# byronknoll/gmix

Measured on AMD Instinct MI355X. Metric: mixer bits/sec (synthetic 256-input mixer streams, forward+update), higher is better.
Workload: dtype f32; 1 GPU; configs[1]: synthetic 256-input 1-layer mixer (1 mixer, 2^16-row gate table), random logits, forward+update; n_inputs=256, mixers=1/0/0, streams_per_gpu=4096, total_bits=5486149632, parallelism=streams sharded over 1 GPU(s), no collective on the data path

## Files before the change

gmix_amd/csrc/gmx_capi.cpp:

```cpp
#include <hip/hip_runtime.h>
#include <math.h>
#include <stdio.h>
#include <stdlib.h>
#include <string.h>
#include <time.h>

#include <algorithm>
#include <atomic>
#include <map>
#include <new>
#include <string>
#include <vector>

#include "../../include/gmxmix.h"
#include "gmx_buildhash.h"
#include "gmx_internal.h"
#include "gmx_ckpt.h"
#include "gmx_ind_ckpt.h"
#include "gmx_match.h"
#include "gmx_match_ckpt.h"

struct GmxSynthArgs {
  float* pred;
  uint32_t* mask;
  uint32_t* ctx;
  uint8_t* bits;
  uint64_t* rng;
  uint64_t* tcount;
  float* pstate;
  uint32_t* cstate;
  uint64_t rec_stride, n_bits, seed;
  int32_t n, n_pad, m, mask_words, n_streams, restart, ctx_mode, bit_mode;
  uint32_t ctx_mod, zero_mod;
};

extern "C" {
hipError_t gmx_launch_bank_kernel(const GmxTopoDev* tp_dev, const GmxRunArgs* args, int n_streams,
                                  unsigned lds_bytes, int has_mask, int l0, int l1, int ns, int fin,
                                  unsigned stride0, hipStream_t stream);
hipError_t gmx_bank_kernel_set_lds(unsigned lds_bytes);
int gmx_bank_kernel_build(int l0, int l1, int ns, int fin, unsigned stride0);
hipError_t gmx_launch_stock_kernel(const GmxTopoDev* tp_dev, const GmxRunArgs* args, int n_streams,
                                   unsigned lds_bytes, int has_mask, int staged, int pow2_tables, hipStream_t stream);
hipError_t gmx_launch_single_kernel(const GmxTopoDev* tp_dev, const GmxRunArgs* args, int n_inputs,
                                    int variant, hipStream_t stream);
hipError_t gmx_launch_wide_kernel(const GmxTopoDev* tp_dev, const GmxRunArgs* args, int n_streams, int has_mask,
                                  int n_inputs, hipStream_t stream);
hipError_t gmx_launch_pair_kernel(const GmxTopoDev* tp_dev, const GmxRunArgs* args, int n_streams, int has_mask,
                                  int n_inputs, int l0, int l1, hipStream_t stream);
int gmx_pair_kernel_half(int n_inputs);
hipError_t gmx_launch_synth_kernel(const GmxSynthArgs* args, hipStream_t stream);
struct GmxDecayArgs {
  const uint64_t* steps0;
  float* table;
  uint32_t* amb;
  uint32_t amb_cap, U;
  uint64_t T;
};
hipError_t gmx_launch_decay_kernel(const GmxDecayArgs* args, hipStream_t stream);
hipError_t gmx_launch_init_scal(uint8_t* banks, uint64_t bank_bytes, uint64_t scal_off, int m,
                                int n_streams, hipStream_t stream);
hipError_t gmx_launch_math_probe(const float* x, float* y, uint64_t n, int what, hipStream_t stream);
hipError_t gmx_launch_math_range(uint64_t lo, uint64_t count, int what, unsigned long long* out,
                                 hipStream_t stream);
}

static thread_local std::string g_last_error;

static int hip_fail(hipError_t e, const char* what) {
  char buf[512];
  snprintf(buf, sizeof buf, "%s: %s (%d)", what, hipGetErrorString(e), (int)e);
  g_last_error = buf;
  (void)hipGetLastError();
  return GMX_ERR_HIP;
}
#define HIPCHK(call)                                   \
  do {                                                 \
    hipError_t e_ = (call);                            \
    if (e_ != hipSuccess) return hip_fail(e_, #call);  \
  } while (0)

static const size_t kBatchOwnStreamMin = 256u * 1024u;
struct GmxXfer {
  hipEvent_t ev_up = nullptr;
  hipEvent_t ev_dev = nullptr;
  hipEvent_t ev_down = nullptr;
  hipEvent_t ev_wr = nullptr;
  bool up_rec = false, dev_rec = false, down_rec = false, wr_rec = false;
  bool idle = false;
};
static int xfer_init(GmxXfer& x) {
  HIPCHK(hipEventCreateWithFlags(&x.ev_up, hipEventDisableTiming));
  HIPCHK(hipEventCreateWithFlags(&x.ev_dev, hipEventDisableTiming));
  HIPCHK(hipEventCreateWithFlags(&x.ev_down, hipEventDisableTiming));
  HIPCHK(hipEventCreateWithFlags(&x.ev_wr, hipEventDisableTiming));
  return GMX_OK;
}
static void xfer_free(GmxXfer& x) {
  hipEvent_t evs[] = {x.ev_up, x.ev_dev, x.ev_down, x.ev_wr};
  for (hipEvent_t e : evs)
    if (e) (void)hipEventDestroy(e);
  x = GmxXfer();
}
static int xfer_note_device_use(GmxXfer& x, hipStream_t main) {
  HIPCHK(hipEventRecord(x.ev_dev, main));
  x.dev_rec = true;
  x.idle = false;
  return GMX_OK;
}
static int xfer_writer_waits(GmxXfer& x, hipStream_t writer) {
  if (x.up_rec) HIPCHK(hipStreamWaitEvent(writer, x.ev_up, 0));
  if (x.dev_rec) HIPCHK(hipStreamWaitEvent(writer, x.ev_dev, 0));
  if (x.wr_rec) HIPCHK(hipStreamWaitEvent(writer, x.ev_wr, 0));
  return GMX_OK;
}
static int xfer_writer_done(GmxXfer& x, hipStream_t writer, hipStream_t main) {
  HIPCHK(hipEventRecord(x.ev_wr, writer));
  x.wr_rec = true;
  x.idle = false;
  HIPCHK(hipStreamWaitEvent(main, x.ev_wr, 0));
  return GMX_OK;
}
static hipError_t bank_stream_create(hipStream_t* out, int level ) {
  int least = 0, greatest = 0;
  hipError_t e = hipDeviceGetStreamPriorityRange(&least, &greatest);
  if (e != hipSuccess) return e;
  const int mid = (least + greatest) / 2;
  return hipStreamCreateWithPriority(out, hipStreamNonBlocking, level == 1 ? least : level == 2 ? greatest : mid);
}
static hipError_t sibling_stream_create(hipStream_t* out, hipStream_t main) {
// ... 83 lines not shown
  const int k = (int)(c.seq++ % (unsigned)kStageSlots);
  if (c.busy[k]) {
    HIPCHK(hipEventSynchronize(c.done[k]));
    c.busy[k] = false;
  }
  if ((size_t)n > c.cap) {
    for (int j = 0; j < kStageSlots; ++j) {
      if (c.busy[j]) {
        HIPCHK(hipEventSynchronize(c.done[j]));
        c.busy[j] = false;
      }
      if (c.dev[j]) (void)hipFree(c.dev[j]);
      if (c.host[j]) (void)hipHostFree(c.host[j]);
      c.dev[j] = nullptr;
      c.host[j] = nullptr;
    }
    c.cap = 0;
    const size_t cap = (size_t)n + 64;
    for (int j = 0; j < kStageSlots; ++j) {
      HIPCHK(hipMalloc((void**)&c.dev[j], cap * sizeof(uint64_t)));
      HIPCHK(hipHostMalloc((void**)&c.host[j], cap * sizeof(uint64_t), hipHostMallocDefault));
      if (!c.done[j]) HIPCHK(hipEventCreateWithFlags(&c.done[j], hipEventDisableTiming));
    }
    c.cap = cap;
  }
  memcpy(c.host[k], counts, (size_t)n * sizeof(uint64_t));
  HIPCHK(hipMemcpyAsync(c.dev[k], c.host[k], (size_t)n * sizeof(uint64_t), hipMemcpyHostToDevice, st));
  *dev_out = c.dev[k];
  return GMX_OK;
}
static int count_list_used(GmxCountList& c, hipStream_t st) {
  const int k = (int)((c.seq - 1u) % (unsigned)kStageSlots);
  HIPCHK(hipEventRecord(c.done[k], st));
  c.busy[k] = true;
  return GMX_OK;
}

struct gmx_group {
  int device = 0;
  int S = 0;
  GmxTopoDev topo;
  GmxTopoDev* topo_dev = nullptr;
  uint8_t* banks = nullptr;
  float* latch_out = nullptr;
  hipStream_t stream = nullptr;
  hipEvent_t ev0 = nullptr, ev1 = nullptr;
  unsigned lds_bytes = 0;
  std::vector<uint64_t> steps;
  std::vector<uint8_t> fwd_done;
  struct DecaySlot {
    float* dev = nullptr;
    uint32_t* idx_dev = nullptr;
    float* host = nullptr;
    uint32_t* idx_host = nullptr;
    size_t cap = 0;
    size_t idx_cap = 0;
    hipEvent_t done = nullptr;
    hipEvent_t ready = nullptr;
    bool busy = false;
    uint64_t* st_dev = nullptr;
    uint64_t* st_host = nullptr;
    uint32_t* amb_dev = nullptr;
    uint32_t* amb_host = nullptr;
    float* patch_host = nullptr;
    size_t st_cap = 0;
  } decay[kStageSlots];
  GmxCountList counts;
  hipStream_t copy_stream = nullptr;
  hipStream_t up_stream = nullptr, down_stream = nullptr;
  unsigned run_seq = 0;
  hipEvent_t tm0 = nullptr, tm1 = nullptr;
  gmx_batch* one = nullptr;
  std::vector<gmx_batch*> batches;
  std::vector<struct GmxSession*> sessions;
  std::vector<struct gmx_lockstep*> locksteps;
  bool banks_in_use_by_dead_kernel = false;
  bool use_sessions = true;
  bool mailbox_on_device = true;
  bool force_general = false;
  bool stock_exact = false;
  int stock_staged = -1;
  bool decay_on_host = false;
  bool stock_pairs = false;
  bool register_rows = false;
  int single_variant = 0;
  struct GmxCkptState* ckpt = nullptr;
};

struct gmx_batch {
  gmx_group* g = nullptr;
  int S = 0;
  uint64_t max_bits = 0;
  unsigned flags = 0;
  float* d_pred = nullptr;
  uint32_t* d_mask = nullptr;
  uint32_t* d_ctx = nullptr;
  uint8_t* d_bits = nullptr;
  float* d_p = nullptr;
  float* d_out = nullptr;
  float* d_last = nullptr;
  uint64_t* d_rng = nullptr;
  uint64_t* d_tcount = nullptr;
  float* d_pstate = nullptr;
  uint32_t* d_cstate = nullptr;
  float* h_pred = nullptr;
  uint32_t* h_mask = nullptr;
  uint32_t* h_ctx = nullptr;
  uint8_t* h_bits = nullptr;
  float* h_p = nullptr;
  float* h_out = nullptr;
  float* h_last = nullptr;
  GmxXfer x;
};

struct gmx_lockstep {
  gmx_group* g = nullptr;
  gmx_batch* b = nullptr;
  float* dec_host = nullptr;
  uint8_t* bits_host = nullptr;
  float* dec_dev = nullptr;
  uint32_t* idx_dev = nullptr;
  hipGraph_t g_predict = nullptr, g_learn = nullptr, g_step = nullptr;
  hipGraphExec_t x_predict = nullptr, x_learn = nullptr, x_step = nullptr;
  bool predicted = false;
  bool persistent = false, ps_running = false, ps_dead = false, ps_counted = false;
  hipStream_t ps_stream = nullptr;
  GmxLsDoor* door = nullptr;
  uint32_t* done = nullptr;
  uint32_t* blk_seen = nullptr;
  uint32_t* blk_replay = nullptr;
  uint32_t* relay = nullptr;
  float* live = nullptr;
  uint32_t seq = 0, word = 0, completed = 0;
  bool learn_inflight = false;
};

enum GmxKernelKind : int;
static GmxKernelKind kernel_for(const gmx_group* g, unsigned mode);
static int sessions_close(gmx_group* g, bool keep_forward);
static int locksteps_stop(gmx_group* g, gmx_lockstep* except, bool keep_forward);
static void sessions_free(gmx_group* g);
static void ckpt_free(gmx_group* g);

extern "C" const char* gmx_strerror(int status) {
  switch (status) {
    case GMX_OK: return "ok";
    case GMX_ERR_INVALID: return "invalid argument or unsupported topology";
    case GMX_ERR_NOMEM: return "out of memory";
    case GMX_ERR_HIP: return "HIP runtime error";
    case GMX_ERR_NO_DEVICE: return "no usable gfx950 device (this library has no CPU fallback)";
    case GMX_ERR_STATE: return "call order violated";
    case GMX_ERR_FORMAT: return "malformed checkpoint";
    default: return "unknown status";
  }
}

extern "C" const char* gmx_last_error(void) { return g_last_error.c_str(); }

extern "C" const char* gmx_build_info(void) {
  return "libgmxmix gfx950 (CDNA4) hipcc -O3 -ffp-contract=off; abi 1; src " GMX_SRC_HASH "; kernels " GMX_KERN_HASH;
}

extern "C" int gmx_device_count(int* count) {
  if (!count) return GMX_ERR_INVALID;
  int n = 0;
  hipError_t e = hipGetDeviceCount(&n);
// ... 392 lines not shown
    on_device = rcd == GMX_OK;
  }
  if (!on_device) {
    for (auto& kv : uniq) {
      float* tab = d.host + (size_t)kv.second * T;
      if (learn)
        for (uint64_t t = 0; t < T; ++t) tab[t] = decay_base(kv.first + t);
      else
        for (uint64_t t = 0; t < T; ++t) tab[t] = 0.f;
    }
    HIPCHK(hipMemcpyAsync(d.dev, d.host, uniq.size() * T * sizeof(float), hipMemcpyHostToDevice, g->copy_stream));
  }
  memcpy(d.idx_host, idx.data(), ns * sizeof(uint32_t));
  HIPCHK(hipMemcpyAsync(d.idx_dev, d.idx_host, ns * sizeof(uint32_t), hipMemcpyHostToDevice, g->copy_stream));
  HIPCHK(hipEventRecord(d.ready, g->copy_stream));
  HIPCHK(hipStreamWaitEvent(g->stream, d.ready, 0));
  return GMX_OK;
}

static bool topo_register_rows_eligible(const GmxTopoDev& t) {
  return t.has_final && t.l0 >= 1 && t.l0 <= 24 && t.l1 >= 1 && t.l1 <= 8 && t.m == t.l0 + t.l1 + 1 &&
         t.n_skip == 1 && gmx_pair_kernel_half(t.n) != 0;
}

enum GmxKernelKind : int { GMX_K_SINGLE, GMX_K_WIDE, GMX_K_STOCK, GMX_K_BANK, GMX_K_PAIR };
static GmxKernelKind kernel_for(const gmx_group* g, unsigned mode) {
  if (g->register_rows && (mode & GMX_MODE_PREDICT) && !(mode & GMX_MODE_LATCH) && !g->force_general &&
      topo_register_rows_eligible(g->topo))
    return GMX_K_PAIR;
  const bool single = g->topo.m == 1 && g->topo.n <= 256 && (mode & GMX_MODE_PREDICT) &&
                      !(mode & GMX_MODE_LATCH) && !g->force_general;
  const bool stock = g->topo.n == 90 && g->topo.l0 == 24 && g->topo.l1 == 8 && g->topo.n_skip == 1 &&
                     g->topo.has_final && g->topo.mx[23].stride == 128 && !g->force_general;
  const bool wide = g->topo.l0 == 24 && g->topo.l1 == 8 && g->topo.n_skip == 1 && g->topo.has_final &&
                    ((g->topo.n == 256 && g->topo.mx[23].stride == 288) ||
                     (g->topo.n == 90 && g->topo.mx[23].stride == 128 && g->stock_pairs && !g->stock_exact)) &&
                    (mode & GMX_MODE_PREDICT) && !(mode & GMX_MODE_LATCH) && !g->force_general;
  return single ? GMX_K_SINGLE : wide ? GMX_K_WIDE : stock ? GMX_K_STOCK : GMX_K_BANK;
}

static int launch_run(gmx_group* g, gmx_batch* b, int s0, int rec0, int ns, uint64_t T,
                      unsigned mode, float* kernel_ms, const uint64_t* n_list = nullptr) {
  if (T == 0) return GMX_OK;
  for (gmx_lockstep* ls : g->locksteps) ls->predicted = false;
  gmx_group::DecaySlot* dec = nullptr;
  int rc = prepare_decay(g, s0, ns, T, (mode & GMX_MODE_LEARN) ? 1 : 0, &dec);
  if (rc) return rc;
  GmxRunArgs a;
  memset(&a, 0, sizeof a);
  a.banks = g->banks;
  a.pred = b->d_pred;
  a.mask = (b->flags & GMX_BATCH_MASK) ? b->d_mask : nullptr;
  a.ctx = b->d_ctx;
  a.bits = b->d_bits;
  a.decay = dec->dev;
  a.decay_idx = dec->idx_dev;
  a.p_out = b->d_p;
  a.out_all = (b->flags & GMX_BATCH_OUTPUTS) ? b->d_out : nullptr;
  a.out_last = (b->flags & GMX_BATCH_LAST_OUTPUTS) ? b->d_last : nullptr;
  a.latch_out = g->latch_out;
  a.rec_stride = b->max_bits;
  a.T = T;
  if (n_list) {
    int rcl = count_list_stage(g->counts, n_list, ns, g->stream, &a.T_list);
    if (rcl) return rcl;
  }
  a.mode = mode | (g->stock_exact ? GMX_MODE_EXACT : 0u);
  a.stream_base = s0;
  a.rec_base = rec0;
  a.n_streams = ns;
  {
    int rcx = xfer_before_run(b->x, g->stream);
    if (rcx) return rcx;
  }
  if (kernel_ms) HIPCHK(hipEventRecord(g->ev0, g->stream));
  const GmxKernelKind kind = kernel_for(g, mode);
  const bool single = kind == GMX_K_SINGLE, wide = kind == GMX_K_WIDE, stock = kind == GMX_K_STOCK;
  if (a.out_last && (single || wide)) return GMX_ERR_INVALID;
  if (kind == GMX_K_PAIR)
    HIPCHK(gmx_launch_pair_kernel(g->topo_dev, &a, ns, a.mask != nullptr, g->topo.n, g->topo.l0, g->topo.l1, g->stream));
  else if (single)
    HIPCHK(gmx_launch_single_kernel(g->topo_dev, &a, g->topo.n, g->single_variant, g->stream));
  else if (wide)
    HIPCHK(gmx_launch_wide_kernel(g->topo_dev, &a, ns, a.mask != nullptr, g->topo.n, g->stream));
  else if (stock)
    HIPCHK(gmx_launch_stock_kernel(g->topo_dev, &a, ns, GMX_STK_LDS_BYTES(g->topo.lds_misc),
                                   a.mask != nullptr, g->stock_staged, topo_tables_pow2(g->topo), g->stream));
  else
    HIPCHK(gmx_launch_bank_kernel(g->topo_dev, &a, ns, g->lds_bytes, a.mask != nullptr, g->topo.l0,
                                  g->topo.l1, g->topo.n_skip, g->topo.has_final,
                                  g->topo.mx[g->topo.l0 - 1].stride, g->stream));
  HIPCHK(hipEventRecord(dec->done, g->stream));
  dec->busy = true;
  if (n_list) {
    int rcl = count_list_used(g->counts, g->stream);
    if (rcl) return rcl;
  }
  {
    int rcn = batch_note_device_use(b);
    if (rcn) return rcn;
  }
  if (kernel_ms) {
    HIPCHK(hipEventRecord(g->ev1, g->stream));
    HIPCHK(hipEventSynchronize(g->ev1));
    HIPCHK(hipEventElapsedTime(kernel_ms, g->ev0, g->ev1));
  }
  if (mode & GMX_MODE_LEARN)
    for (int i = 0; i < ns; ++i) g->steps[s0 + i] += n_list ? n_list[i] : T;
  return GMX_OK;
}

static void batch_free(gmx_batch* b) {
  if (!b) return;
  if (b->g) {
    (void)hipSetDevice(b->g->device);
    if (b->g->stream) (void)hipStreamSynchronize(b->g->stream);
    if (b->g->up_stream) (void)hipStreamSynchronize(b->g->up_stream);
    if (b->g->down_stream) (void)hipStreamSynchronize(b->g->down_stream);
    auto& v = b->g->batches;
    v.erase(std::remove(v.begin(), v.end(), b), v.end());
  }
  void* dv[] = {b->d_pred, b->d_mask, b->d_ctx, b->d_bits, b->d_p, b->d_out, b->d_last,
                b->d_rng, b->d_tcount, b->d_pstate, b->d_cstate};
  for (void* p : dv)
    if (p) (void)hipFree(p);
  void* hv[] = {b->h_pred, b->h_mask, b->h_ctx, b->h_bits, b->h_p, b->h_out, b->h_last};
  for (void* p : hv)
    if (p) (void)hipHostFree(p);
  xfer_free(b->x);
  delete b;
}

static int batch_alloc(gmx_batch** out, gmx_group* g, int S, uint64_t max_bits, unsigned flags) {
  if (!out || !g || max_bits == 0) return GMX_ERR_INVALID;
  *out = nullptr;
  HIPCHK(hipSetDevice(g->device));
  gmx_batch* b = new (std::nothrow) gmx_batch();
  if (!b) return GMX_ERR_NOMEM;
  b->g = g;
  b->S = S;
  b->max_bits = max_bits;
  b->flags = flags;
  const GmxTopoDev& t = g->topo;
  const size_t R = (size_t)S * max_bits;
#define BCHK(call)                                 \
  do {                                             \
    hipError_t e_ = (call);                        \
    if (e_ != hipSuccess) {                        \
      int r_ = hip_fail(e_, #call);                \
      batch_free(b);                               \
      return e_ == hipErrorOutOfMemory ? GMX_ERR_NOMEM : r_; \
    }                                              \
  } while (0)
  BCHK(hipMalloc((void**)&b->d_pred, R * t.n_pad * sizeof(float)));
  if (flags & GMX_BATCH_MASK) BCHK(hipMalloc((void**)&b->d_mask, R * t.mask_words * sizeof(uint32_t)));
  BCHK(hipMalloc((void**)&b->d_ctx, (R + 1) * t.m * sizeof(uint32_t)));
  BCHK(hipMalloc((void**)&b->d_bits, R));
  BCHK(hipMalloc((void**)&b->d_p, R * sizeof(float)));
  if (flags & GMX_BATCH_OUTPUTS) BCHK(hipMalloc((void**)&b->d_out, R * t.m * sizeof(float)));
  if (flags & GMX_BATCH_LAST_OUTPUTS) {
    BCHK(hipMalloc((void**)&b->d_last, (size_t)S * t.m * sizeof(float)));
    BCHK(hipMemset(b->d_last, 0, (size_t)S * t.m * sizeof(float)));
  }
#undef BCHK
  {
    int rcx = xfer_init(b->x);
    if (rcx) {
// ... 371 lines not shown
      memcpy(w + (size_t)r * x.stride, p + 12, 4 * (size_t)input_size);
      p += 12 + 4 * (size_t)input_size;
    }
  }
  if (p != end) return GMX_ERR_FORMAT;
  HIPCHK(hipSetDevice(g->device));
  int rc = sessions_close(g, true);
  if (rc) return rc;
  if (stream < (int)g->sessions.size() && g->sessions[stream]) g->sessions[stream]->fwd_live = false;
  HIPCHK(hipStreamSynchronize(g->stream));
  HIPCHK(hipMemcpy(g->banks + (size_t)stream * t.bank_bytes, img.data(), img.size(),
                   hipMemcpyHostToDevice));
  g->steps[stream] = sc[0];
  g->fwd_done[stream] = 0;
  for (gmx_lockstep* ls : g->locksteps) ls->predicted = false;
  return GMX_OK;
}

extern "C" int gmx_bank_copy(gmx_group* dst, int dst_stream, gmx_group* src, int src_stream) {
  if (!dst || !src || dst_stream < 0 || dst_stream >= dst->S || src_stream < 0 || src_stream >= src->S)
    return GMX_ERR_INVALID;
  const GmxTopoDev &a = dst->topo, &b = src->topo;
  if (a.m != b.m || a.n != b.n || a.n_skip != b.n_skip || a.bank_bytes != b.bank_bytes)
    return GMX_ERR_INVALID;
  for (int j = 0; j < a.m; ++j)
    if (a.mx[j].table_size != b.mx[j].table_size || a.mx[j].weight_size != b.mx[j].weight_size ||
        a.mx[j].layer != b.mx[j].layer)
      return GMX_ERR_INVALID;
  HIPCHK(hipSetDevice(src->device));
  int rc = sessions_close(src, true);
  if (rc) return rc;
  HIPCHK(hipStreamSynchronize(src->stream));
  HIPCHK(hipSetDevice(dst->device));
  rc = sessions_close(dst, true);
  if (rc) return rc;
  if (dst_stream < (int)dst->sessions.size() && dst->sessions[dst_stream])
    dst->sessions[dst_stream]->fwd_live = false;
  HIPCHK(hipStreamSynchronize(dst->stream));
  HIPCHK(hipMemcpy(dst->banks + (size_t)dst_stream * a.bank_bytes,
                   src->banks + (size_t)src_stream * b.bank_bytes, a.bank_bytes,
                   hipMemcpyDeviceToDevice));
  dst->steps[dst_stream] = src->steps[src_stream];
  dst->fwd_done[dst_stream] = 0;
  for (gmx_lockstep* ls : dst->locksteps) ls->predicted = false;
  return GMX_OK;
}

#include "gmx_ckpt.inc"

extern "C" int gmx_bank_memory_usage(gmx_group* g, int stream, int mixer, uint64_t* bytes) {
  if (!g || stream < 0 || stream >= g->S || mixer < 0 || mixer >= g->topo.m || !bytes)
    return GMX_ERR_INVALID;
  HIPCHK(hipSetDevice(g->device));
  int rc = sessions_close(g, true);
  if (rc) return rc;
  HIPCHK(hipStreamSynchronize(g->stream));
  uint64_t sc[3];
  HIPCHK(hipMemcpy(sc, g->banks + (size_t)stream * g->topo.bank_bytes + g->topo.scal_off + 24u * mixer,
                   24, hipMemcpyDeviceToHost));
  const GmxMixerDev& x = g->topo.mx[mixer];
  *bytes = 29 + sc[2] * (uint64_t)(x.weight_size * 4 + 12) + 8ull * x.table_size;
  return GMX_OK;
}


#include "gmx_indirect.inc"
#include "gmx_ind_ckpt.inc"
#include "gmx_lstm.inc"
#include "gmx_match.inc"
#include "gmx_match_ckpt.inc"
#include "gmx_chainstep.inc"

extern "C" int gmx_debug_single_variant(gmx_group* g, int lanes_per_stream) {
  if (!g || (lanes_per_stream != 0 && lanes_per_stream != 16 && lanes_per_stream != 32 &&
             lanes_per_stream != 64 && lanes_per_stream != 165 && lanes_per_stream != 325))
    return GMX_ERR_INVALID;
  g->single_variant = lanes_per_stream;
  return GMX_OK;
}

extern "C" int gmx_debug_stock_pairs(gmx_group* g, int on) {
  if (!g) return GMX_ERR_INVALID;
  g->stock_pairs = on != 0;
  return GMX_OK;
}

extern "C" int gmx_debug_decay_on_host(gmx_group* g, int on) {
  if (!g) return GMX_ERR_INVALID;
  g->decay_on_host = on != 0;
  return GMX_OK;
}

extern "C" int gmx_debug_decay_table(gmx_group* g, const uint64_t* steps0, int U, uint64_t T, float* out,
                                     uint32_t* n_unsettled) {
  if (!g || !steps0 || U < 1 || T < 1 || !out) return GMX_ERR_INVALID;
  HIPCHK(hipSetDevice(g->device));
  if (!g->copy_stream) HIPCHK(sibling_stream_create(&g->copy_stream, g->stream));
  gmx_group::DecaySlot tmp;
  std::map<uint64_t, uint32_t> uniq;
  std::vector<uint32_t> row(U);
  for (int u = 0; u < U; ++u) {
    auto it = uniq.find(steps0[u]);
    if (it == uniq.end()) it = uniq.emplace(steps0[u], (uint32_t)uniq.size()).first;
    row[u] = it->second;
  }
  HIPCHK(hipMalloc((void**)&tmp.dev, uniq.size() * T * sizeof(float)));
  int rc = decay_table_on_device(g, tmp, uniq, T);
  if (rc == GMX_OK) {
    if (n_unsettled) *n_unsettled = tmp.amb_host[0];
    std::vector<float> h(uniq.size() * T);
    hipError_t e = hipMemcpyAsync(h.data(), tmp.dev, h.size() * sizeof(float), hipMemcpyDeviceToHost, g->copy_stream);
    if (e == hipSuccess) e = hipStreamSynchronize(g->copy_stream);
    if (e != hipSuccess) rc = hip_fail(e, "gmx_debug_decay_table copy");
    else
      for (int u = 0; u < U; ++u) memcpy(out + (size_t)u * T, h.data() + (size_t)row[u] * T, T * sizeof(float));
  }
  void* dv[] = {tmp.dev, tmp.st_dev, tmp.amb_dev};
  for (void* p : dv)
    if (p) (void)hipFree(p);
  void* hv[] = {tmp.st_host, tmp.amb_host, tmp.patch_host};
  for (void* p : hv)
    if (p) (void)hipHostFree(p);
  return rc;
}

extern "C" int gmx_topology_register_rows_eligible(const gmx_topology* topo) {
  GmxTopoDev td;
  if (build_topology(topo, &td) != GMX_OK) return GMX_ERR_INVALID;
  return topo_register_rows_eligible(td) ? 1 : 0;
}

extern "C" int gmx_group_set_register_rows(gmx_group* g, int on) {
  if (!g || !topo_register_rows_eligible(g->topo)) return GMX_ERR_INVALID;
  g->register_rows = on != 0;
  return GMX_OK;
}

extern "C" int gmx_debug_force_general(gmx_group* g, int on) {
  if (!g) return GMX_ERR_INVALID;
  g->force_general = on != 0;
  return GMX_OK;
}

extern "C" int gmx_debug_kernel_kind(gmx_group* g, unsigned mode) {
  if (!g) return GMX_ERR_INVALID;
  const GmxKernelKind kind = kernel_for(g, mode);
  if (kind != GMX_K_BANK) return (int)kind;
  const GmxTopoDev& t = g->topo;
  return (int)kind + 4 * gmx_bank_kernel_build(t.l0, t.l1, t.n_skip, t.has_final, t.mx[t.l0 - 1].stride);
}

extern "C" int gmx_debug_stock_staged(gmx_group* g, int mode) {
  if (!g || mode < -1 || mode > 1) return GMX_ERR_INVALID;
  g->stock_staged = mode;
  return GMX_OK;
}

extern "C" int gmx_debug_stock_exact(gmx_group* g, int on) {
  if (!g) return GMX_ERR_INVALID;
  int rc = sessions_close(g, true);
  if (rc) return rc;
  g->stock_exact = on != 0;
  return GMX_OK;
}

extern "C" int gmx_debug_use_sessions(gmx_group* g, int on) {
// ... 404 lines not shown
```

gmix_amd/csrc/gmx_wide.hip:

```cpp
#include <hip/hip_runtime.h>
#include <stdint.h>

#include "gmx_internal.h"
#include "gmx_math.h"

typedef float gmx_f4 __attribute__((ext_vector_type(4)));

namespace {

constexpr int kL0 = 24, kL1 = 8, kM = kL0 + kL1 + 1;
constexpr int kQS = 9;
constexpr int kFinLane = 56;
constexpr int kPitchS = 4 * kQS + 4;

template <int N, int HALF>
struct WideShape {
  static constexpr int kN = N, kHalf = HALF;
  static constexpr int kNPad = (N + 3) / 4 * 4;
  static constexpr int kMW = (N + 31) / 32;
  static constexpr int kQ = HALF / 4;
  static constexpr int kUp = N - HALF;
  static constexpr int kQU = (kUp + 3) / 4;
  static constexpr int kPitch = HALF + 4;
  static constexpr int kStageSmall = 2 * kL0 * kPitch;
  static constexpr int kStageFloats = kStageSmall + (kL1 + 1) * kPitchS;
  static_assert(HALF % 4 == 0 && HALF <= N && N - HALF + kL0 - 1 <= HALF, "layer-0 rows must split into two lanes");
  static_assert((kPitch / 4) % 2 == 1, "odd quad pitch keeps the transposed reads conflict-free");
  static constexpr int stage_off(int h) {
    return h < kL0 ? h * kPitch
           : h < 32 ? kStageSmall + (h - kL0) * kPitchS
           : h < 32 + kL0 ? (kL0 + h - 32) * kPitch
           : h == kFinLane ? kStageSmall + kL1 * kPitchS : 0;
  }
  static constexpr int stage_lanes(int h) {
    return h < kL0 ? kQ : (h >= 32 && h < 32 + kL0) ? (kUp + (h - 32) + 3) / 4 : ((h < 32 || h == kFinLane) ? kQS : 0);
  }
};

__device__ __forceinline__ void wide_ld16(gmx_f4& d, const void* p) {
  asm volatile("global_load_dwordx4 %0, %1, off nt" : "=v"(d) : "v"(p) : "memory");
}
__device__ __forceinline__ void wide_ld4(uint32_t& d, const void* p) {
  asm volatile("global_load_dword %0, %1, off" : "=v"(d) : "v"(p) : "memory");
}
__device__ __forceinline__ void wide_ld1(uint32_t& d, const void* p) {
  asm volatile("global_load_ubyte %0, %1, off" : "=v"(d) : "v"(p) : "memory");
}
__device__ __forceinline__ uint32_t readlane_u(uint32_t v, int l) {
  return (uint32_t)__builtin_amdgcn_readlane((int)v, l);
}
__device__ __forceinline__ uint32_t wide_lds_addr(const void* p) {
  return (uint32_t)(uintptr_t)(__attribute__((address_space(3))) const void*)p;
}
__device__ __forceinline__ void wide_dma16(uint64_t sbase, uint32_t voff, uint32_t lds_byte, uint64_t mask) {
  uint32_t sm0;
  asm volatile(
      "s_mov_b64 exec, %3\n\ts_mov_b32 %0, m0\n\ts_mov_b32 m0, %4\n\ts_nop 0\n\t"
      "global_load_lds_dwordx4 %2, %1 nt\n\ts_mov_b32 m0, %0\n\ts_mov_b64 exec, -1"
      : "=&s"(sm0)
      : "s"(sbase), "v"(voff), "s"(mask), "s"(lds_byte)
      : "memory");
}
__device__ __forceinline__ void wide_st16(uint64_t sbase, uint32_t voff, const gmx_f4& v, uint64_t mask) {
  asm volatile(
      "s_mov_b64 exec, %3\n\t"
      "global_store_dwordx4 %1, %2, %0 nt\n\ts_mov_b64 exec, -1"
      :
      : "s"(sbase), "v"(voff), "v"(v), "s"(mask)
      : "memory");
}
__device__ __forceinline__ float readlane_f(float v, int l) {
  return __int_as_float(__builtin_amdgcn_readlane(__float_as_int(v), l));
}
__device__ __forceinline__ float el(const gmx_f4& v, int e) { return e == 0 ? v.x : (e == 1 ? v.y : (e == 2 ? v.z : v.w)); }

}

template <int N, int HALF, bool HAS_MASK>
__global__ void __launch_bounds__(64) __attribute__((amdgpu_waves_per_eu(1, 2)))
gmx_wide_kernel(const GmxTopoDev* __restrict__ tp, const GmxRunArgs a) {
  using SH = WideShape<N, HALF>;
  constexpr int kHalf = SH::kHalf, kNPad = SH::kNPad, kMW = SH::kMW, kQ = SH::kQ, kUp = SH::kUp,
                kQU = SH::kQU, kPitch = SH::kPitch, kStageSmall = SH::kStageSmall;
  __shared__ __attribute__((aligned(16))) float xin[kNPad + 4];
  __shared__ __attribute__((aligned(16))) float stage[SH::kStageFloats];
  __shared__ uint64_t s_tab[32];
  const int lane = threadIdx.x;
  const int rec = a.rec_base + (int)blockIdx.x;
  const int s = a.stream_base + (int)blockIdx.x;
  const uint64_t T = a.T;
  if (T == 0) return;
  if (lane < 32) s_tab[lane] = gmx_exp2f_tab[lane];
  for (int i = 4 * lane; i < SH::kStageFloats; i += 256) *(gmx_f4*)(stage + i) = gmx_f4{0.f, 0.f, 0.f, 0.f};
  const bool do_learn = (a.mode & GMX_MODE_LEARN) != 0;
  uint8_t* const bank = a.banks + (uint64_t)s * tp->bank_bytes;

  const int half = lane >> 5, li = lane & 31;
  const bool is_l0 = li < kL0;
  const bool is_l1 = half == 0 && li >= kL0;
  const bool is_fin = lane == kFinLane;
  const bool act = is_l0 || is_l1 || is_fin;
  const bool owner = act && !(is_l0 && half);
  const int mxi = is_fin ? kM - 1 : (act ? li : 0);
  const int k1 = li - kL0;
  const GmxMixerDev d = tp->mx[mxi];
  const int skip_idx = tp->skip_idx[0];
  const bool all_pow2 = __ballot(act && (d.table_size & (d.table_size - 1u)) != 0) == 0;
  uint64_t* const scal = (uint64_t*)(bank + tp->scal_off) + 3 * mxi;
  uint64_t steps = 0, max_steps = 1, seen_cnt = 0;
  if (act) {
    steps = scal[0];
    max_steps = scal[1];
    seen_cnt = scal[2];
  }
  constexpr bool kFolded = true;
  uint64_t* const rs_tab = (uint64_t*)(bank + d.rs_off);
  uint8_t* const w_tab = bank + d.w_off + ((is_l0 && half) ? kHalf * 4u : 0u);
  const uint32_t row_bytes = d.stride * 4u;

  const uint64_t RS = a.rec_stride;
  const float* const pred_s = a.pred + (uint64_t)rec * RS * kNPad;
  const uint32_t* const mask_s = HAS_MASK ? a.mask + (uint64_t)rec * RS * kMW : nullptr;
  const uint32_t* const ctx_s = a.ctx + (uint64_t)rec * RS * kM;
  const uint8_t* const bits_s = a.bits + (uint64_t)rec * RS;
  const float* const dec_s = a.decay + (uint64_t)a.decay_idx[blockIdx.x] * T;
  float* const p_s = a.p_out + (uint64_t)rec * RS;
  float* const oa_s = a.out_all ? a.out_all + (uint64_t)rec * RS * kM : nullptr;

  gmx_f4 w[kQ];
#pragma unroll
  for (int q = 0; q < kQ; ++q) w[q] = gmx_f4{0.f, 0.f, 0.f, 0.f};
  uint32_t tag = 0xffffffffu;
  uint64_t rs = 0;
  bool dirty = false;

  float* const my_stage = stage + (is_l0 ? (half * kL0 + li) * kPitch
                                                        : kStageSmall + (is_fin ? kL1 : (li - kL0)) * kPitchS);
  const uint32_t stage_base = wide_lds_addr(stage);
  const uint32_t lane16 = (uint32_t)lane * 16u;
  auto evict = [&](bool ev) {
    const uint64_t em = __ballot(ev);
    if (em == 0) return;
    const uint64_t dst = (uint64_t)(w_tab + (uint64_t)tag * row_bytes);
    const uint32_t dlo = (uint32_t)dst, dhi = (uint32_t)(dst >> 32);
    if (ev) {
#pragma unroll
      for (int q = 0; q < kQS; ++q) *(gmx_f4*)(my_stage + 4 * q) = w[q];
      if (owner) *(kFolded ? (uint64_t*)((uint8_t*)rs_tab + (uint64_t)tag * row_bytes) : rs_tab + tag) = rs;
    }
    if (ev && is_l0) {
#pragma unroll
      for (int q = kQS; q < kQ; ++q) *(gmx_f4*)(my_stage + 4 * q) = w[q];
    }
#pragma unroll
    for (int h = 0; h <= kFinLane; ++h) {
      if (SH::stage_lanes(h) == 0) continue;
      const uint64_t m = ((em >> h) & 1u) ? ((1ull << SH::stage_lanes(h)) - 1ull) : 0ull;
      const uint64_t sb = ((uint64_t)readlane_u(dhi, h) << 32) | readlane_u(dlo, h);
      const gmx_f4 v = *(const gmx_f4*)(stage + SH::stage_off(h) + 4 * (lane < SH::stage_lanes(h) ? lane : 0));
      wide_st16(sb, lane16, v, m);
    }
  };
  auto fetch = [&](uint64_t nm, uint64_t src) {
    const uint32_t slo = (uint32_t)src, shi = (uint32_t)(src >> 32);
#pragma unroll
    for (int h = 0; h <= kFinLane; ++h) {
      if (SH::stage_lanes(h) == 0) continue;
      const uint64_t m = ((nm >> h) & 1u) ? ((1ull << SH::stage_lanes(h)) - 1ull) : 0ull;
      const uint64_t sb = ((uint64_t)readlane_u(shi, h) << 32) | readlane_u(slo, h);
      wide_dma16(sb, lane16, stage_base + (uint32_t)SH::stage_off(h) * 4u, m);
    }
  };

  uint32_t ctx_n = 0, mask_n = ~0u, bit_n = 0, dec_n = 0;
  gmx_f4 x_n = gmx_f4{0.f, 0.f, 0.f, 0.f};
  auto request = [&](uint64_t t) {
    const uint64_t tt = t < T ? t : T - 1;
    wide_ld4(ctx_n, ctx_s + tt * (uint64_t)kM + mxi);
    wide_ld16(x_n, pred_s + tt * (uint64_t)kNPad + 4 * (4 * lane < kNPad ? lane : 0));
    if (HAS_MASK) wide_ld4(mask_n, mask_s + tt * (uint64_t)kMW + (lane < kMW ? lane : 0));
    wide_ld1(bit_n, bits_s + tt);
    wide_ld4(dec_n, dec_s + tt);
  };
  auto landed = [&]() {
    asm volatile("s_waitcnt vmcnt(0)" : "+v"(ctx_n), "+v"(x_n), "+v"(mask_n), "+v"(bit_n), "+v"(dec_n));
  };
  request(0);
  landed();

  for (uint64_t t = 0; t < T; ++t) {
    const uint32_t ctx = ctx_n, mword = mask_n, bit = bit_n & 1u;
    const float dec = __uint_as_float(dec_n);
    const gmx_f4 xv = x_n;

    const uint32_t row = all_pow2 ? (ctx & (d.table_size - 1u)) : (ctx % d.table_size);
    const bool need = act && row != tag;
    evict(need && dirty);
    const uint64_t nm = __ballot(need);
    if (nm) {
      fetch(nm, (uint64_t)(w_tab + (uint64_t)row * row_bytes));
      if (need) rs = *(kFolded ? (const uint64_t*)((const uint8_t*)rs_tab + (uint64_t)row * row_bytes) : rs_tab + row);
      asm volatile("s_waitcnt vmcnt(0)" : "+v"(rs) : : "memory");
      if (need) {
#pragma unroll
        for (int q = 0; q < kQS; ++q) w[q] = *(const gmx_f4*)(my_stage + 4 * q);
        tag = row;
        dirty = false;
      }
      if (need && is_l0) {
#pragma unroll
        for (int q = kQS; q < kQ; ++q) w[q] = *(const gmx_f4*)(my_stage + 4 * q);
      }
    }
    request(t + 1);

    const bool has_x = 4 * lane < kNPad;
    if (has_x) *(gmx_f4*)(xin + 4 * lane) = xv;
    const float skip = xin[skip_idx];
    if (HAS_MASK) {
      const uint32_t word = (uint32_t)__builtin_amdgcn_ds_bpermute((has_x ? (lane >> 3) : 0) << 2, (int)mword);
      const uint32_t b = word >> ((4u * (uint32_t)lane) & 31u);
      gmx_f4 v = xv;
      v.x = (b & 1u) ? v.x : 0.f;
      v.y = (b & 2u) ? v.y : 0.f;
      v.z = (b & 4u) ? v.z : 0.f;
      v.w = (b & 8u) ? v.w : 0.f;
      if (has_x) *(gmx_f4*)(xin + 4 * lane) = v;
    }
    const bool seen = act && rs != 0;

    float acc = 0.f;
#pragma unroll
    for (int q = 0; q < kQ; ++q) {
      const gmx_f4 x = *(const gmx_f4*)(xin + 4 * q);
      acc = acc + x.x * w[q].x;
      acc = acc + x.y * w[q].y;
      acc = acc + x.z * w[q].z;
      acc = acc + x.w * w[q].w;
    }
    acc = __int_as_float(__builtin_amdgcn_ds_bpermute(((lane & 31)) << 2, __float_as_int(acc)));
#pragma unroll
    for (int q = 0; q < kQU; ++q) {
      const gmx_f4 x = *(const gmx_f4*)(xin + kHalf + 4 * q);
      if (4 * q + 0 < kUp) acc = acc + x.x * w[q].x;
      if (4 * q + 1 < kUp) acc = acc + x.y * w[q].y;
      if (4 * q + 2 < kUp) acc = acc + x.z * w[q].z;
      if (4 * q + 3 < kUp) acc = acc + x.w * w[q].w;
    }
    acc = seen ? acc : 0.f;
    float o0[kL0];
    const bool up0 = is_l0 && half && seen;
#pragma unroll
    for (int i = 0; i < kL0; ++i) {
      o0[i] = readlane_f(acc, 32 + i);
      if (i + 1 < kL0) {
        const float wt = el(w[(kUp + i) / 4], (kUp + i) % 4);
        acc = (up0 && li > i) ? acc + o0[i] * wt : acc;
      }
    }
    const bool up1 = (is_l1 || is_fin) && seen;
    float a1 = 0.f;
#pragma unroll
    for (int i = 0; i < kL0; ++i) a1 = a1 + o0[i] * el(w[i / 4], i % 4);
    a1 = up1 ? a1 : 0.f;
    float o1[kL1];
#pragma unroll
    for (int i = 0; i < kL1; ++i) {
      const float wt = el(w[(kL0 + i) / 4], (kL0 + i) % 4);
      a1 = (is_l1 && k1 == i && seen) ? a1 + skip * wt : a1;
      o1[i] = readlane_f(a1, kL0 + i);
      a1 = (((is_l1 && k1 > i) || is_fin) && seen) ? a1 + o1[i] * wt : a1;
    }
    a1 = (is_fin && seen) ? a1 + skip * w[(kL0 + kL1) / 4].x : a1;
    static_assert((kL0 + kL1) % 4 == 0, "the final mixer's skip weight is element 0 of its quad");

    const float own0 = __int_as_float(__builtin_amdgcn_ds_bpermute((32 + (lane & 31)) << 2, __float_as_int(acc)));
    const float own = is_l0 ? own0 : a1;
    const float pl = gmx_logistic_tab(own, s_tab);
    if (is_fin) p_s[t] = gmx_clamp_prob(pl);
    if (oa_s && owner) oa_s[t * (uint64_t)kM + mxi] = own;

    if (do_learn) {
      const double dd = (double)dec * (1.5 - ((double)rs) / (double)max_steps);
      const float decay = (float)dd;
      const float upd = decay * d.lr * (pl - (float)bit);
      const uint64_t rs_new = rs + 1;
      const float scl = ((rs_new & 1023u) == 0) ? (1.0f - 3.0e-6f) : 1.0f;
      if (act) {
        ++steps;
        if (rs_new > max_steps) max_steps = rs_new;
        if (rs == 0) ++seen_cnt;
        rs = rs_new;
        dirty = true;
      }
#pragma unroll
      for (int q = 0; q < kQ; ++q) {
        const gmx_f4 xl = *(const gmx_f4*)(xin + 4 * q);
        gmx_f4 xh = gmx_f4{0.f, 0.f, 0.f, 0.f};
        if (4 * q < kUp) xh = *(const gmx_f4*)(xin + kHalf + 4 * q);
        float c[4];
#pragma unroll
        for (int e = 0; e < 4; ++e) {
          const int j = 4 * q + e;
          const int i = j - kUp;
          c[e] = j < kUp ? el(xh, e) : ((i + 1 < kL0 && li > i) ? o0[(i >= 0 && i < kL0) ? i : 0] : 0.f);
        }
        gmx_f4 x;
        x.x = half ? c[0] : xl.x;
        x.y = half ? c[1] : xl.y;
        x.z = half ? c[2] : xl.z;
        x.w = half ? c[3] : xl.w;
        if (q < kQS) {
          float sm[4];
#pragma unroll
          for (int e = 0; e < 4; ++e) {
            const int idx = 4 * q + e;
            float v = 0.f;
            if (idx < kL0) {
              v = o0[idx];
            } else if (idx < kL0 + kL1) {
              const int i = idx - kL0;
              v = (is_fin || k1 > i) ? o1[i] : (k1 == i ? skip : 0.f);
            } else if (idx == kL0 + kL1) {
              v = is_fin ? skip : 0.f;
            }
            sm[e] = v;
          }
          x.x = is_l0 ? x.x : sm[0];
          x.y = is_l0 ? x.y : sm[1];
          x.z = is_l0 ? x.z : sm[2];
          x.w = is_l0 ? x.w : sm[3];
        } else {
          x.x = is_l0 ? x.x : 0.f;
          x.y = is_l0 ? x.y : 0.f;
          x.z = is_l0 ? x.z : 0.f;
          x.w = is_l0 ? x.w : 0.f;
        }
        w[q].x = (w[q].x - upd * x.x) * scl;
        w[q].y = (w[q].y - upd * x.y) * scl;
        w[q].z = (w[q].z - upd * x.z) * scl;
        w[q].w = (w[q].w - upd * x.w) * scl;
      }
    }
    landed();
  }
  evict(act && dirty);
  if (owner && do_learn) {
    scal[0] = steps;
    scal[1] = max_steps;
    scal[2] = seen_cnt;
  }
}

extern "C" hipError_t gmx_launch_wide_kernel(const GmxTopoDev* tp_dev, const GmxRunArgs* args, int n_streams,
                                             int has_mask, int n_inputs, hipStream_t stream) {
  (void)hipGetLastError();
  const dim3 grid(n_streams), block(64);
  if (n_inputs == 256) {
    if (has_mask)
      hipLaunchKernelGGL((gmx_wide_kernel<256, 144, true>), grid, block, 0, stream, tp_dev, *args);
    else
      hipLaunchKernelGGL((gmx_wide_kernel<256, 144, false>), grid, block, 0, stream, tp_dev, *args);
  } else if (n_inputs == 90) {
    if (has_mask)
      hipLaunchKernelGGL((gmx_wide_kernel<90, 64, true>), grid, block, 0, stream, tp_dev, *args);
    else
      hipLaunchKernelGGL((gmx_wide_kernel<90, 64, false>), grid, block, 0, stream, tp_dev, *args);
  } else {
    return hipErrorInvalidValue;
  }
  return hipGetLastError();
}
```

Measured before the change: 1.837 billion bits/s.

## Split wide-kernel layer-0 staging into double-buffered quarter parts for two waves per SIMD

Adds a PARTS template parameter to the 256-input wide kernel. With four parts, layer-0 row staging in LDS shrinks to two rotating quarter buffers, so two waves fit per SIMD. Row fetches are pipelined part by part with partial vmcnt waits, and evictions are batched in small groups. The quartered variant is picked automatically when streams exceed the SIMD count. The cost is more wait/sync bookkeeping, a masked rs load, and a tighter register budget, which could cause spills.

```diff
diff --git a/gmix_amd/csrc/gmx_capi.cpp b/gmix_amd/csrc/gmx_capi.cpp
--- a/gmix_amd/csrc/gmx_capi.cpp
+++ b/gmix_amd/csrc/gmx_capi.cpp
@@ -45,7 +45,7 @@
 hipError_t gmx_launch_single_kernel(const GmxTopoDev* tp_dev, const GmxRunArgs* args, int n_inputs,
                                     int variant, hipStream_t stream);
 hipError_t gmx_launch_wide_kernel(const GmxTopoDev* tp_dev, const GmxRunArgs* args, int n_streams, int has_mask,
-                                  int n_inputs, hipStream_t stream);
+                                  int n_inputs, int image, hipStream_t stream);
 hipError_t gmx_launch_pair_kernel(const GmxTopoDev* tp_dev, const GmxRunArgs* args, int n_streams, int has_mask,
                                   int n_inputs, int l0, int l1, hipStream_t stream);
 int gmx_pair_kernel_half(int n_inputs);
@@ -295,6 +295,7 @@
   int stock_staged = -1;
   bool decay_on_host = false;
   bool stock_pairs = false;
+  int wide_image = 0;
   bool register_rows = false;
   int single_variant = 0;
   struct GmxCkptState* ckpt = nullptr;
@@ -853,7 +854,7 @@
   else if (single)
     HIPCHK(gmx_launch_single_kernel(g->topo_dev, &a, g->topo.n, g->single_variant, g->stream));
   else if (wide)
-    HIPCHK(gmx_launch_wide_kernel(g->topo_dev, &a, ns, a.mask != nullptr, g->topo.n, g->stream));
+    HIPCHK(gmx_launch_wide_kernel(g->topo_dev, &a, ns, a.mask != nullptr, g->topo.n, g->wide_image, g->stream));
   else if (stock)
     HIPCHK(gmx_launch_stock_kernel(g->topo_dev, &a, ns, GMX_STK_LDS_BYTES(g->topo.lds_misc),
                                    a.mask != nullptr, g->stock_staged, topo_tables_pow2(g->topo), g->stream));
@@ -1391,6 +1392,12 @@
 extern "C" int gmx_debug_stock_pairs(gmx_group* g, int on) {
   if (!g) return GMX_ERR_INVALID;
   g->stock_pairs = on != 0;
+  return GMX_OK;
+}
+
+extern "C" int gmx_debug_wide_image(gmx_group* g, int parts) {
+  if (!g || (parts != 0 && parts != 1 && parts != 4)) return GMX_ERR_INVALID;
+  g->wide_image = parts;
   return GMX_OK;
 }
 
diff --git a/gmix_amd/csrc/gmx_wide.hip b/gmix_amd/csrc/gmx_wide.hip
--- a/gmix_amd/csrc/gmx_wide.hip
+++ b/gmix_amd/csrc/gmx_wide.hip
@@ -12,8 +12,9 @@
 constexpr int kQS = 9;
 constexpr int kFinLane = 56;
 constexpr int kPitchS = 4 * kQS + 4;
-
-template <int N, int HALF>
+constexpr int kEvictGroup = 6;
+
+template <int N, int HALF, int PARTS>
 struct WideShape {
   static constexpr int kN = N, kHalf = HALF;
   static constexpr int kNPad = (N + 3) / 4 * 4;
@@ -22,14 +23,26 @@
   static constexpr int kUp = N - HALF;
   static constexpr int kQU = (kUp + 3) / 4;
   static constexpr int kPitch = HALF + 4;
-  static constexpr int kStageSmall = 2 * kL0 * kPitch;
+  static constexpr int kParts = PARTS;
+  static constexpr int kRowsP = 2 * kL0 / PARTS;
+  static constexpr int kBufFloats = kRowsP * kPitch;
+  static constexpr int kStageSmall = (PARTS > 1 ? 2 : 1) * kBufFloats;
   static constexpr int kStageFloats = kStageSmall + (kL1 + 1) * kPitchS;
   static_assert(HALF % 4 == 0 && HALF <= N && N - HALF + kL0 - 1 <= HALF, "layer-0 rows must split into two lanes");
   static_assert((kPitch / 4) % 2 == 1, "odd quad pitch keeps the transposed reads conflict-free");
+  static_assert(PARTS == 1 || (PARTS % 2 == 0 && kL0 % (PARTS / 2) == 0), "a part lies within the lower or the upper halves");
+  static constexpr int l0_lane(int i) { return i < kL0 ? i : 32 + i - kL0; }
+  static constexpr int part_lane(int k, int r) { return l0_lane(k * kRowsP + r); }
+  static constexpr uint64_t part_mask(int k) {
+    uint64_t m = 0;
+    for (int r = 0; r < kRowsP; ++r) m |= 1ull << part_lane(k, r);
+    return m;
+  }
+  static constexpr int l0_off(int i) { return ((i / kRowsP) & 1) * kBufFloats + (i % kRowsP) * kPitch; }
   static constexpr int stage_off(int h) {
-    return h < kL0 ? h * kPitch
+    return h < kL0 ? l0_off(h)
            : h < 32 ? kStageSmall + (h - kL0) * kPitchS
-           : h < 32 + kL0 ? (kL0 + h - 32) * kPitch
+           : h < 32 + kL0 ? l0_off(kL0 + h - 32)
            : h == kFinLane ? kStageSmall + kL1 * kPitchS : 0;
   }
   static constexpr int stage_lanes(int h) {
@@ -69,6 +82,14 @@
       : "s"(sbase), "v"(voff), "v"(v), "s"(mask)
       : "memory");
 }
+__device__ __forceinline__ void wide_ld8_masked(uint64_t& d, const void* p, uint64_t mask) {
+  asm volatile(
+      "s_mov_b64 exec, %2\n\t"
+      "global_load_dwordx2 %0, %1, off\n\ts_mov_b64 exec, -1"
+      : "+v"(d)
+      : "v"(p), "s"(mask)
+      : "memory");
+}
 __device__ __forceinline__ float readlane_f(float v, int l) {
   return __int_as_float(__builtin_amdgcn_readlane(__float_as_int(v), l));
 }
@@ -76,10 +97,10 @@
 
 }
 
-template <int N, int HALF, bool HAS_MASK>
-__global__ void __launch_bounds__(64) __attribute__((amdgpu_waves_per_eu(1, 2)))
+template <int N, int HALF, int PARTS, bool HAS_MASK>
+__global__ void __launch_bounds__(64) __attribute__((amdgpu_waves_per_eu(PARTS > 1 ? 2 : 1, 2)))
 gmx_wide_kernel(const GmxTopoDev* __restrict__ tp, const GmxRunArgs a) {
-  using SH = WideShape<N, HALF>;
+  using SH = WideShape<N, HALF, PARTS>;
   constexpr int kHalf = SH::kHalf, kNPad = SH::kNPad, kMW = SH::kMW, kQ = SH::kQ, kUp = SH::kUp,
                 kQU = SH::kQU, kPitch = SH::kPitch, kStageSmall = SH::kStageSmall;
   __shared__ __attribute__((aligned(16))) float xin[kNPad + 4];
@@ -91,7 +112,9 @@
   const uint64_t T = a.T;
   if (T == 0) return;
   if (lane < 32) s_tab[lane] = gmx_exp2f_tab[lane];
-  for (int i = 4 * lane; i < SH::kStageFloats; i += 256) *(gmx_f4*)(stage + i) = gmx_f4{0.f, 0.f, 0.f, 0.f};
+  if constexpr (PARTS == 1) {
+    for (int i = 4 * lane; i < SH::kStageFloats; i += 256) *(gmx_f4*)(stage + i) = gmx_f4{0.f, 0.f, 0.f, 0.f};
+  }
   const bool do_learn = (a.mode & GMX_MODE_LEARN) != 0;
   uint8_t* const bank = a.banks + (uint64_t)s * tp->bank_bytes;
 
@@ -134,41 +157,73 @@
   uint64_t rs = 0;
   bool dirty = false;
 
-  float* const my_stage = stage + (is_l0 ? (half * kL0 + li) * kPitch
-                                                        : kStageSmall + (is_fin ? kL1 : (li - kL0)) * kPitchS);
+  constexpr int kParts = SH::kParts, kRowsP = SH::kRowsP;
+  const int my_row = kL0 * half + li;
+  const int my_part = is_l0 ? my_row / kRowsP : -1;
+  float* const my_stage = stage + (is_l0 ? ((my_row / kRowsP) & 1) * SH::kBufFloats + (my_row % kRowsP) * kPitch
+                                         : kStageSmall + (is_fin ? kL1 : (li - kL0)) * kPitchS);
   const uint32_t stage_base = wide_lds_addr(stage);
   const uint32_t lane16 = (uint32_t)lane * 16u;
+  constexpr uint64_t kSmallLanes = (((1ull << kL1) - 1ull) << kL0) | (1ull << kFinLane);
   auto evict = [&](bool ev) {
     const uint64_t em = __ballot(ev);
     if (em == 0) return;
     const uint64_t dst = (uint64_t)(w_tab + (uint64_t)tag * row_bytes);
     const uint32_t dlo = (uint32_t)dst, dhi = (uint32_t)(dst >> 32);
-    if (ev) {
-#pragma unroll
-      for (int q = 0; q < kQS; ++q) *(gmx_f4*)(my_stage + 4 * q) = w[q];
-      if (owner) *(kFolded ? (uint64_t*)((uint8_t*)rs_tab + (uint64_t)tag * row_bytes) : rs_tab + tag) = rs;
-    }
-    if (ev && is_l0) {
-#pragma unroll
-      for (int q = kQS; q < kQ; ++q) *(gmx_f4*)(my_stage + 4 * q) = w[q];
-    }
-#pragma unroll
-    for (int h = 0; h <= kFinLane; ++h) {
-      if (SH::stage_lanes(h) == 0) continue;
-      const uint64_t m = ((em >> h) & 1u) ? ((1ull << SH::stage_lanes(h)) - 1ull) : 0ull;
-      const uint64_t sb = ((uint64_t)readlane_u(dhi, h) << 32) | readlane_u(dlo, h);
-      const gmx_f4 v = *(const gmx_f4*)(stage + SH::stage_off(h) + 4 * (lane < SH::stage_lanes(h) ? lane : 0));
-      wide_st16(sb, lane16, v, m);
-    }
-  };
-  auto fetch = [&](uint64_t nm, uint64_t src) {
-    const uint32_t slo = (uint32_t)src, shi = (uint32_t)(src >> 32);
-#pragma unroll
-    for (int h = 0; h <= kFinLane; ++h) {
-      if (SH::stage_lanes(h) == 0) continue;
-      const uint64_t m = ((nm >> h) & 1u) ? ((1ull << SH::stage_lanes(h)) - 1ull) : 0ull;
-      const uint64_t sb = ((uint64_t)readlane_u(shi, h) << 32) | readlane_u(slo, h);
-      wide_dma16(sb, lane16, stage_base + (uint32_t)SH::stage_off(h) * 4u, m);
+    if constexpr (PARTS == 1) {
+      if (ev) {
+#pragma unroll
+        for (int q = 0; q < kQS; ++q) *(gmx_f4*)(my_stage + 4 * q) = w[q];
+        if (owner) *(kFolded ? (uint64_t*)((uint8_t*)rs_tab + (uint64_t)tag * row_bytes) : rs_tab + tag) = rs;
+      }
+      if (ev && is_l0) {
+#pragma unroll
+        for (int q = kQS; q < kQ; ++q) *(gmx_f4*)(my_stage + 4 * q) = w[q];
+      }
+#pragma unroll
+      for (int h = 0; h <= kFinLane; ++h) {
+        if (SH::stage_lanes(h) == 0) continue;
+        const uint64_t m = ((em >> h) & 1u) ? ((1ull << SH::stage_lanes(h)) - 1ull) : 0ull;
+        const uint64_t sb = ((uint64_t)readlane_u(dhi, h) << 32) | readlane_u(dlo, h);
+        const gmx_f4 v = *(const gmx_f4*)(stage + SH::stage_off(h) + 4 * (lane < SH::stage_lanes(h) ? lane : 0));
+        wide_st16(sb, lane16, v, m);
+      }
+      return;
+    }
+    auto store_rows = [&](auto lane_of, int n) {
+#pragma unroll
+      for (int i0 = 0; i0 < n; i0 += kEvictGroup) {
+        gmx_f4 v[kEvictGroup];
+#pragma unroll
+        for (int i = 0; i < kEvictGroup; ++i) {
+          const int h = lane_of(i0 + i < n ? i0 + i : 0);
+          if (i0 + i < n) v[i] = *(const gmx_f4*)(stage + SH::stage_off(h) + 4 * (lane < SH::stage_lanes(h) ? lane : 0));
+        }
+#pragma unroll
+        for (int i = 0; i < kEvictGroup; ++i) {
+          const int h = lane_of(i0 + i < n ? i0 + i : 0);
+          const uint64_t m = ((em >> h) & 1u) ? ((1ull << SH::stage_lanes(h)) - 1ull) : 0ull;
+          const uint64_t sb = ((uint64_t)readlane_u(dhi, h) << 32) | readlane_u(dlo, h);
+          if (i0 + i < n) wide_st16(sb, lane16, v[i], m);
+        }
+      }
+    };
+    if (ev && owner) *(kFolded ? (uint64_t*)((uint8_t*)rs_tab + (uint64_t)tag * row_bytes) : rs_tab + tag) = rs;
+    if (em & kSmallLanes) {
+      if (ev && !is_l0) {
+#pragma unroll
+        for (int q = 0; q < kQS; ++q) *(gmx_f4*)(my_stage + 4 * q) = w[q];
+      }
+      store_rows([](int i) { return i < kL1 ? kL0 + i : kFinLane; }, kL1 + 1);
+    }
+#pragma unroll
+    for (int k = 0; k < kParts; ++k) {
+      if ((em & SH::part_mask(k)) == 0) continue;
+      if (ev && my_part == k) {
+#pragma unroll
+        for (int q = 0; q < kQ; ++q) *(gmx_f4*)(my_stage + 4 * q) = w[q];
+      }
+      store_rows([k](int i) { return SH::part_lane(k, i); }, kRowsP);
     }
   };
 
@@ -197,23 +252,84 @@
     const bool need = act && row != tag;
     evict(need && dirty);
     const uint64_t nm = __ballot(need);
-    if (nm) {
-      fetch(nm, (uint64_t)(w_tab + (uint64_t)row * row_bytes));
-      if (need) rs = *(kFolded ? (const uint64_t*)((const uint8_t*)rs_tab + (uint64_t)row * row_bytes) : rs_tab + row);
-      asm volatile("s_waitcnt vmcnt(0)" : "+v"(rs) : : "memory");
-      if (need) {
+    const uint64_t src = (uint64_t)(w_tab + (uint64_t)row * row_bytes);
+    const uint32_t slo = (uint32_t)src, shi = (uint32_t)(src >> 32);
+    auto fetch_row = [&](int h) {
+      const uint64_t m = ((nm >> h) & 1u) ? ((1ull << SH::stage_lanes(h)) - 1ull) : 0ull;
+      const uint64_t sb = ((uint64_t)readlane_u(shi, h) << 32) | readlane_u(slo, h);
+      wide_dma16(sb, lane16, stage_base + (uint32_t)SH::stage_off(h) * 4u, m);
+    };
+    auto fetch_part = [&](int k) {
+#pragma unroll
+      for (int r = 0; r < kRowsP; ++r) fetch_row(SH::part_lane(k, r));
+    };
+    auto take_part = [&](int k) {
+      if (need && my_part == k) {
+        const int pieces = half ? (kUp + li + 3) / 4 : kQ;
+#pragma unroll
+        for (int q = 0; q < kQ; ++q) {
+          gmx_f4 v = *(const gmx_f4*)(my_stage + 4 * q);
+          if ((k + 1) * kRowsP > kL0 && q >= (kUp + 3) / 4) v = q < pieces ? v : gmx_f4{0.f, 0.f, 0.f, 0.f};
+          w[q] = v;
+        }
+      }
+    };
+    auto take_small = [&]() {
+      if (need && !is_l0) {
 #pragma unroll
         for (int q = 0; q < kQS; ++q) w[q] = *(const gmx_f4*)(my_stage + 4 * q);
-        tag = row;
-        dirty = false;
-      }
-      if (need && is_l0) {
-#pragma unroll
-        for (int q = kQS; q < kQ; ++q) w[q] = *(const gmx_f4*)(my_stage + 4 * q);
-      }
-    }
-    request(t + 1);
-
+      }
+    };
+    if constexpr (PARTS == 1) {
+      if (nm) {
+#pragma unroll
+        for (int h = 0; h <= kFinLane; ++h) {
+          if (SH::stage_lanes(h) != 0) fetch_row(h);
+        }
+        if (need) rs = *(kFolded ? (const uint64_t*)((const uint8_t*)rs_tab + (uint64_t)row * row_bytes) : rs_tab + row);
+        asm volatile("s_waitcnt vmcnt(0)" : "+v"(rs) : : "memory");
+        if (need) {
+#pragma unroll
+          for (int q = 0; q < kQS; ++q) w[q] = *(const gmx_f4*)(my_stage + 4 * q);
+          tag = row;
+          dirty = false;
+        }
+        if (need && is_l0) {
+#pragma unroll
+          for (int q = kQS; q < kQ; ++q) w[q] = *(const gmx_f4*)(my_stage + 4 * q);
+        }
+      }
+      request(t + 1);
+    } else {
+      if (nm) {
+        wide_ld8_masked(rs, kFolded ? (const void*)((const uint8_t*)rs_tab + (uint64_t)row * row_bytes) : (const void*)(rs_tab + row), nm);
+  #pragma unroll
+        for (int h = kL0; h < 32; ++h) fetch_row(h);
+        fetch_row(kFinLane);
+        fetch_part(0);
+        fetch_part(1);
+  #pragma unroll
+        for (int k = 0; k + 1 < kParts; ++k) {
+          asm volatile("s_waitcnt vmcnt(%1)" : "+v"(rs) : "n"(kRowsP) : "memory");
+          if (k == 0) take_small();
+          take_part(k);
+          if (k + 2 < kParts) {
+            asm volatile("s_waitcnt lgkmcnt(0)" : : : "memory");
+            fetch_part(k + 2);
+          }
+        }
+      }
+      request(t + 1);
+      if (nm) {
+        asm volatile("s_waitcnt vmcnt(%1)" : "+v"(rs) : "n"(4 + (HAS_MASK ? 1 : 0)) : "memory");
+        take_part(kParts - 1);
+        if (need) {
+          tag = row;
+          dirty = false;
+        }
+      }
+
+    }
     const bool has_x = 4 * lane < kNPad;
     if (has_x) *(gmx_f4*)(xin + 4 * lane) = xv;
     const float skip = xin[skip_idx];
@@ -353,19 +469,35 @@
 }
 
 extern "C" hipError_t gmx_launch_wide_kernel(const GmxTopoDev* tp_dev, const GmxRunArgs* args, int n_streams,
-                                             int has_mask, int n_inputs, hipStream_t stream) {
+                                             int has_mask, int n_inputs, int image, hipStream_t stream) {
   (void)hipGetLastError();
   const dim3 grid(n_streams), block(64);
   if (n_inputs == 256) {
-    if (has_mask)
-      hipLaunchKernelGGL((gmx_wide_kernel<256, 144, true>), grid, block, 0, stream, tp_dev, *args);
-    else
-      hipLaunchKernelGGL((gmx_wide_kernel<256, 144, false>), grid, block, 0, stream, tp_dev, *args);
+    static int simds = 0;
+    if (image == 0 && simds == 0) {
+      int dev = 0, cus = 0;
+      if (hipGetDevice(&dev) != hipSuccess ||
+          hipDeviceGetAttribute(&cus, hipDeviceAttributeMultiprocessorCount, dev) != hipSuccess || cus <= 0)
+        return hipErrorInvalidDevice;
+      simds = 4 * cus;
+    }
+    const bool quarters = image ? image == 4 : n_streams > simds;
+    if (quarters) {
+      if (has_mask)
+        hipLaunchKernelGGL((gmx_wide_kernel<256, 144, 4, true>), grid, block, 0, stream, tp_dev, *args);
+      else
+        hipLaunchKernelGGL((gmx_wide_kernel<256, 144, 4, false>), grid, block, 0, stream, tp_dev, *args);
+    } else {
+      if (has_mask)
+        hipLaunchKernelGGL((gmx_wide_kernel<256, 144, 1, true>), grid, block, 0, stream, tp_dev, *args);
+      else
+        hipLaunchKernelGGL((gmx_wide_kernel<256, 144, 1, false>), grid, block, 0, stream, tp_dev, *args);
+    }
   } else if (n_inputs == 90) {
     if (has_mask)
-      hipLaunchKernelGGL((gmx_wide_kernel<90, 64, true>), grid, block, 0, stream, tp_dev, *args);
+      hipLaunchKernelGGL((gmx_wide_kernel<90, 64, 1, true>), grid, block, 0, stream, tp_dev, *args);
     else
-      hipLaunchKernelGGL((gmx_wide_kernel<90, 64, false>), grid, block, 0, stream, tp_dev, *args);
+      hipLaunchKernelGGL((gmx_wide_kernel<90, 64, 1, false>), grid, block, 0, stream, tp_dev, *args);
   } else {
     return hipErrorInvalidValue;
   }
```

Result: no change. 1.837 billion bits/s, median of 2 (-0.0%).
